# qwerty35/lsc_planner

Hardware: AMD Instinct MI355X
Metric: agent-replans/sec (whole node) (higher is better)
Workload: dtype f64

## Files before the change

### include/lsc_planner_amd.h

```cpp
#ifndef LSC_PLANNER_AMD_H
#define LSC_PLANNER_AMD_H

#include <stddef.h>
#include <stdint.h>

#ifdef __cplusplus
extern "C" {
#endif

#ifndef LSC_SEGMENTS
#define LSC_SEGMENTS 5
#endif
#define LSC_M LSC_SEGMENTS
#define LSC_DEG 5
#define LSC_NC 6
#define LSC_SEGV (LSC_M * LSC_NC)
#define LSC_NV (3 * LSC_SEGV)

#define LSC_OK 0
#define LSC_EINVAL (-1)
#define LSC_ENODEV (-2)
#define LSC_ENOMEM (-3)
#define LSC_EHIP (-4)
#define LSC_ESTATE (-5)
// ... 133 lines not shown

int lsc_gjk_batch(lsc_ctx *ctx, const double *pts, int count, double *v, double *dist);

int lsc_kernel_time_ms(lsc_ctx *ctx, int which, double *avg_ms, long *launches);
int lsc_set_timing(lsc_ctx *ctx, int enabled);
int lsc_kernel_times_ms(lsc_ctx *ctx, int which, double *out_ms, long capacity, long *launches);

int lsc_last_goals(lsc_ctx *ctx, float *goals);
int lsc_goal_storage(lsc_ctx *ctx, int *where);

int lsc_set_goal_trace(lsc_ctx *ctx, int path_cap);
int lsc_get_goal_trace(lsc_ctx *ctx, int *path_cells, int *path_len, int *flags, int *expansions, int grid_dims[3],
                       double grid_min[3]);

int lsc_last_row_counts(lsc_ctx *ctx, int *rows);
int lsc_neighbour_counts(lsc_ctx *ctx, int *units, int *priority_candidates);
int lsc_row_capacity(const lsc_ctx *ctx, int *lds_rows, int *throughput_rows);
int lsc_last_bucket_max(lsc_ctx *ctx, int *rows);

int lsc_iterations_total(lsc_ctx *ctx, long long *total, int reset);
int lsc_row_iterations_total(lsc_ctx *ctx, long long *total);

int lsc_solver_stats(lsc_ctx *ctx, long long out[4]);

int lsc_phase_profile(lsc_ctx *ctx, int enable, long long *out);
int lsc_goal_profile(lsc_ctx *ctx, int enable, long long *out);
int lsc_goal_key_table(int words, unsigned int *out, int *rank_bits);
int lsc_general_profile(lsc_ctx *ctx, long long *out);
int lsc_solver_residuals(lsc_ctx *ctx, double *out);
int lsc_dump_qp(lsc_ctx *ctx, int agent, const char *path);
int lsc_solver_trace(lsc_ctx *ctx, int agent, double *out);

#ifdef __cplusplus
}
#endif
#endif
```

### lsc_planner_amd/_lib.py

```python
import ctypes
import os

_HERE = os.path.dirname(os.path.abspath(__file__))
_LIBS = {}

M, DEG, NC, SEGV, NV = 5, 5, 6, 30, 90


def segments_of(horizon, dt):
    return int((horizon + 1e-9) / dt)

STATUS_OK, STATUS_INFEASIBLE, STATUS_SFC_BLOCKED, STATUS_GOAL_CAPACITY = 0, 1, 4, 5
COMM_ID_BYTES = 128


class LscError(RuntimeError):
    pass


class LscConfig(ctypes.Structure):
    _fields_ = [
        ("dt", ctypes.c_double),
        ("control_weight", ctypes.c_double),
        ("terminal_weight", ctypes.c_double),
# ... 13 lines not shown
        ("grid_resolution", ctypes.c_double),
        ("grid_margin", ctypes.c_double),
        ("horizon", ctypes.c_double),
        ("goal_row_cap", ctypes.c_int),
        ("planner_mode", ctypes.c_int),
        ("slack_mode", ctypes.c_int),
        ("slack_collision_weight", ctypes.c_double),
        ("n_constraint_segments", ctypes.c_int),
        ("reset_threshold", ctypes.c_double),
        ("gap_tolerance", ctypes.c_double),
        ("world_dimension", ctypes.c_int),
        ("world_z_2d", ctypes.c_double),
        ("goal_search", ctypes.c_int),
        ("solver", ctypes.c_int),
        ("goal_lds_row_cap", ctypes.c_int),
    ]


EXPORTS = [
    "lsc_default_config", "lsc_create", "lsc_destroy", "lsc_last_error", "lsc_last_note", "lsc_segments", "lsc_set_agents", "lsc_set_shard",
    "lsc_set_distmap", "lsc_replan_tick", "lsc_tick_device", "lsc_tick_device_fused", "lsc_propagate_device", "lsc_safety_ratio", "lsc_sweep_device", "lsc_sweep_device_f32",
    "lsc_gjk_batch", "lsc_kernel_time_ms", "lsc_kernel_times_ms", "lsc_set_timing", "lsc_last_row_counts", "lsc_iterations_total", "lsc_phase_profile", "lsc_goal_profile", "lsc_goal_key_table", "lsc_general_profile", "lsc_dump_qp", "lsc_solver_residuals", "lsc_solver_trace", "lsc_edt_from_bt", "lsc_free_host", "lsc_last_goals", "lsc_goal_storage", "lsc_set_goal_trace", "lsc_get_goal_trace",
    "lsc_last_bucket_max", "lsc_row_capacity", "lsc_comm_unique_id", "lsc_comm_init", "lsc_comm_info", "lsc_tick_device_sharded", "lsc_replan_tick_all",
    "lsc_row_iterations_total", "lsc_tick_device_fused_batch", "lsc_solver_stats", "lsc_neighbour_counts", "lsc_replan_tick_batch",
    "lsc_flight_weights", "lsc_flight_row_bytes", "lsc_flight_begin", "lsc_flight_reset", "lsc_flight_end", "lsc_fly_device", "lsc_flight_read",
]

FLIGHT_SAMPLES, FLIGHT_SAFETY, FLIGHT_AGENTS = 1, 2, 4
FLIGHT_MAX_TIMES = 64


class LscFlightConfig(ctypes.Structure):
    _fields_ = [("capacity_ticks", ctypes.c_int), ("n_times", ctypes.c_int), ("times", ctypes.c_double * 64), ("what", ctypes.c_int)]


class LscFlightTick(ctypes.Structure):
    _fields_ = [("planner_seq", ctypes.c_int), ("unmet", ctypes.c_int), ("end_unmet", ctypes.c_int), ("moved", ctypes.c_int),
                ("n_status", ctypes.c_int * 6), ("min_ratio", ctypes.c_double), ("pad", ctypes.c_int * 4)]


BUILT_SEGMENTS = (5, 4)


def lib_path(segments=5):
    if segments == 5:
        return os.environ.get("LSC_HIP_LIB") or os.path.join(_HERE, "liblsc_hip.so")
    if segments == 4:
# ... 48 lines not shown
    L.lsc_kernel_times_ms.argtypes = [vp, ctypes.c_int, dp, ctypes.c_long, ctypes.POINTER(ctypes.c_long)]
    L.lsc_set_timing.argtypes = [vp, ctypes.c_int]
    L.lsc_last_row_counts.argtypes = [vp, ip]
    L.lsc_neighbour_counts.argtypes = [vp, ip, ip]
    L.lsc_last_bucket_max.argtypes = [vp, ip]
    L.lsc_row_capacity.argtypes = [vp, ip, ip]
    L.lsc_phase_profile.argtypes = [vp, ctypes.c_int, ctypes.POINTER(ctypes.c_longlong)]
    L.lsc_goal_profile.argtypes = [vp, ctypes.c_int, ctypes.POINTER(ctypes.c_longlong)]
    L.lsc_general_profile.argtypes = [vp, ctypes.POINTER(ctypes.c_longlong)]
    L.lsc_goal_key_table.argtypes = [ctypes.c_int, ctypes.POINTER(ctypes.c_uint), ctypes.POINTER(ctypes.c_int)]
    L.lsc_dump_qp.argtypes = [vp, ctypes.c_int, ctypes.c_char_p]
    L.lsc_solver_residuals.argtypes = [vp, dp]
    L.lsc_solver_trace.argtypes = [vp, ctypes.c_int, dp]
    L.lsc_edt_from_bt.argtypes = [ctypes.c_char_p, fp, fp, ctypes.c_double, ctypes.POINTER(fp), ip, ip, dp]
    L.lsc_last_goals.argtypes = [vp, fp]
    L.lsc_goal_storage.argtypes = [vp, ip]
    L.lsc_set_goal_trace.argtypes = [vp, ctypes.c_int]
    L.lsc_get_goal_trace.argtypes = [vp, ip, ip, ip, ip, ip, dp]
    L.lsc_free_host.argtypes = [vp]
    L.lsc_free_host.restype = None
    L.lsc_iterations_total.argtypes = [vp, ctypes.POINTER(ctypes.c_longlong), ctypes.c_int]
    L.lsc_row_iterations_total.argtypes = [vp, ctypes.POINTER(ctypes.c_longlong)]
    L.lsc_solver_stats.argtypes = [vp, ctypes.POINTER(ctypes.c_longlong)]
    L.lsc_flight_weights.argtypes = [ctypes.c_double, dp, ctypes.c_int, dp, dp, dp, ip]
    L.lsc_flight_row_bytes.argtypes = [ctypes.c_int, ctypes.c_int, ctypes.c_int]
    L.lsc_flight_row_bytes.restype = ctypes.c_size_t
    L.lsc_flight_begin.argtypes = [vp, ctypes.POINTER(LscFlightConfig)]
    L.lsc_flight_reset.argtypes = [vp]
    L.lsc_flight_end.argtypes = [vp]
    L.lsc_fly_device.argtypes = [vp, vpp, vp, vpp, ctypes.c_int, ctypes.c_int, vp, vp, vp, vp]
    L.lsc_flight_read.argtypes = [vp, ctypes.c_int, ctypes.c_int, ctypes.POINTER(LscFlightTick), fp, dp, ip, dp, ip, fp]
    for name in EXPORTS:
        fn = getattr(L, name)
        if fn.restype is ctypes.c_int or name not in ("lsc_default_config", "lsc_create", "lsc_destroy", "lsc_last_error", "lsc_last_note", "lsc_free_host",
                                                      "lsc_flight_row_bytes"):
            fn.restype = ctypes.c_int
    L.lsc_segments.argtypes = []
    if L.lsc_segments() != segments:
        raise LscError(f"{p} plans M = {L.lsc_segments()} segments, not {segments}")
    _LIBS[segments] = L
    return L
```

### lsc_planner_amd/csrc/lsc_abi.cpp

```cpp
#include <hip/hip_runtime.h>
#include <rccl/rccl.h>
#include <dlfcn.h>

#include <cmath>
#include <cstdio>
#include <cstdlib>
#include <cstring>
#include <chrono>
#include <algorithm>
#include <map>
#include <mutex>
#include <string>
#include <unordered_map>
#include <vector>

#include "../../include/lsc_planner_amd.h"
#include "lsc_kernels.h"
#include "lsc_rules.hpp"
#include "lsc_flight.hpp"
#include "lsc_device_mem.hpp"

using namespace lsc;

namespace {
// ... 252 lines not shown
    float *d_state = nullptr, *d_goal = nullptr, *d_prev = nullptr, *d_next = nullptr;
    double *d_cost = nullptr;
    int *d_status = nullptr, *d_iters = nullptr;
    PinnedBuf<float> h_in;
    PinnedBuf<unsigned char> h_out;
    DevBuf<float> d_onormal;
    DevBuf<double> d_od;
    DevBuf<unsigned char> d_spill;
    size_t spill_stride = 0;
    int spill_slots = 0;
    DevBuf<unsigned char> d_ever, d_gen_ws;
    size_t gen_stride = 0;
    int gen_slots = 0;
    DevBuf<unsigned char> d_neigh;
    DevBuf<long long> d_neigh_prof;
    NeighArgs neigh = {};
    DevBuf<unsigned char> d_safety;
    DevBuf<unsigned char> d_flight;
    int flight_capacity = 0, flight_times = 0, flight_what = 0, flight_flown = 0;
    size_t flight_row_bytes = 0;
    hipStream_t flight_stream = nullptr;
    DevBuf<long long> d_goal_prof;
    DevBuf<int> d_goal_path, d_goal_plen;
    MapMem map;
};

static constexpr size_t in_block_floats(size_t n) { return (9 + 3 + NV) * n; }
static constexpr size_t out_block_bytes(size_t rows) { return (sizeof(double) + sizeof(float) * NV + 2 * sizeof(int)) * rows; }
static constexpr size_t FLIGHT_W5 = 0, FLIGHT_W4 = FLIGHT_W5 + 8 * 6 * FLIGHT_MAX_TIMES, FLIGHT_W3 = FLIGHT_W4 + 8 * 5 * FLIGHT_MAX_TIMES,
                        FLIGHT_SEG = FLIGHT_W3 + 8 * 4 * FLIGHT_MAX_TIMES, FLIGHT_HEADER_BYTES = 8192;
static_assert(FLIGHT_SEG + 4 * FLIGHT_MAX_TIMES <= FLIGHT_HEADER_BYTES, "the header holds the tables of 64 record times");
constexpr int TIMED_GROUPS = 7;

struct lsc_ctx {
    lsc_config cfg;
    HostModel hm;
    int N = 0, first = 0, count = 0, cap = 0, cap_tp = 0, n_cu = 256;
    size_t smem_tp = 0;
    std::string err;
    std::string note;
    bool timing = false;
    CtxMem own;
    SwarmMem swarm;
    int last_host_seq = 0;
    bool next_has_all_rows = false;
    bool h_ever_stale = false;
    std::vector<unsigned char> h_ever;
    std::vector<float> h_edt;
    int edt_dims[3] = {0, 0, 0}, edt_kmin[3] = {0, 0, 0};
    double edt_res = 0.0;
    std::vector<double> h_radius;
    int goal_path_cap = 0;
    std::vector<uint32_t> h_fcode;
    int fcode_rb = 0;
    bool goal_profiling = false;
    int grid_dims[3] = {0, 0, 0}, grid_row_cap = 0;
    double grid_min[3] = {0, 0, 0};
    std::vector<int> nb_seq;
    int goal_hbm = 0;
    size_t goal_ws_bytes = 0;
    bool neigh_always = false;
    bool general_handover = false;
    bool generic_lsc_build = false;
    int trace_agent = -1;
    bool profiling = false;
    hipStream_t stream = nullptr;
    std::vector<std::pair<hipEvent_t, hipEvent_t>> ev_pool[TIMED_GROUPS];
    std::vector<double> host_tick_ms;
    size_t ev_used[TIMED_GROUPS] = {0, 0, 0, 0, 0, 0, 0};
    int world = 1, rank = 0, shard_rows = 0, table_rows = 0;
    ncclComm_t comm = nullptr;
};

struct RcclApi {
    void *h = nullptr;
    decltype(&ncclGetUniqueId) GetUniqueId = nullptr;
    decltype(&ncclCommInitRank) CommInitRank = nullptr;
    decltype(&ncclCommDestroy) CommDestroy = nullptr;
    decltype(&ncclAllGather) AllGather = nullptr;
    decltype(&ncclAllReduce) AllReduce = nullptr;
    decltype(&ncclGroupStart) GroupStart = nullptr;
    decltype(&ncclGroupEnd) GroupEnd = nullptr;
    decltype(&ncclGetErrorString) GetErrorString = nullptr;
};

static bool rccl_bind(RcclApi &api);
// ... 230 lines not shown
    if (cap < NBR * (N - 1)) {
        s.spill_stride = plan_spill_bytes(N);
        s.spill_slots = std::min(N, 256);
        HIPCHK(c, s.d_spill.alloc(s.spill_stride * (size_t)s.spill_slots));
    }
    {
        HIPCHK(c, s.d_ever.alloc_zero(n));
        c->h_ever.assign(N, 0);
        const bool general_all = c->cfg.planner_mode == 1 || c->cfg.slack_mode != 0;
        if (general_all || c->cfg.reset_threshold > 0.0) {
            s.gen_stride = general_ws_bytes(N);
            s.gen_slots = std::min(N, 256);
            HIPCHK(c, s.d_gen_ws.alloc(s.gen_stride * (size_t)s.gen_slots));
        }
        c->general_handover = getenv("LSC_GENERAL_HANDOVER") != nullptr;
    }
    {
        c->generic_lsc_build = getenv("LSC_GENERIC_LSC_BUILD") != nullptr;
        const size_t prev = c->note.find("lsc build:");
        if (prev != std::string::npos) c->note.erase(prev >= 2 ? prev - 2 : prev);
        const char *which = c->generic_lsc_build ? "generic pass (LSC_GENERIC_LSC_BUILD)"
                            : (N - 1 > 64 ? "generic pass (more than 64 obstacles)" : "one wave per segment");
        c->note += (c->note.empty() ? "" : "; ") + std::string("lsc build: ") + which;
    }
    HIPCHK(c, s.d_nrows.alloc_zero(n));
    HIPCHK(c, s.d_bmax.alloc_zero(n));
    HIPCHK(c, s.d_order.alloc(n));
    HIPCHK(c, s.d_obs_bound.alloc(4 * n));
    if (N >= NEIGH_MIN_AGENTS && N <= NEIGH_MAX_AGENTS && c->cfg.prune == 1 && !getenv("LSC_NO_NEIGHBOUR_LISTS")) {
        NeighArgs &g = s.neigh;
        c->neigh_always = getenv("LSC_NEIGH_ALWAYS") != nullptr;
        double vm = 0.0, rm = 0.0, dmin = 1e300, dmax = 0.0;
        for (int i = 0; i < N; i++) {
            for (int k = 0; k < 3; k++) vm = std::max(vm, max_vel[3 * i + k]);
            rm = std::max(rm, radius[i]); dmin = std::min(dmin, dw_obs[i]); dmin = std::min(dmin, downwash[i]);
            dmax = std::max(dmax, dw_obs[i]); dmax = std::max(dmax, downwash[i]);
        }
        double cell = vm * M * c->cfg.dt + 4.0 * rm;
        if (const char *e = getenv("LSC_NEIGH_CELL")) { const double v = atof(e); if (v > 0.0) cell = v; }
        if (!(cell > 1e-3)) cell = 1e-3;
        g.sc_max = std::max(1.0, 1.0 / dmin); g.zscale = std::max(1.0, dmax);
        g.inv_cell = 1.0 / cell; g.inv_cell_z = 1.0 / (cell * g.zscale);
        unsigned H = 1024;
        while (H < 4u * (unsigned)N) H <<= 1;
        g.hmask = H - 1; g.ovf_cap = 4096; g.list_cap = 1024; g.plist_cap = NEIGH_PRIO_CAP; g.tag = 0;
        if (const char *e = getenv("LSC_NEIGH_OVF_CAP")) { const int v = atoi(e); if (v >= 1 && v <= 65536) g.ovf_cap = v; }
// ... 395 lines not shown
    a.neigh = c->swarm.neigh.cnt ? &c->swarm.neigh : nullptr;
    a.nv = nullptr;
    a.state = d_state; a.goal = d_goal; a.traj_prev = d_prev;
    a.radius = c->swarm.d_radius; a.radius_obs = c->swarm.d_radius_obs; a.downwash = c->swarm.d_downwash; a.downwash_obs = c->swarm.d_downwash_obs;
    a.vmax = c->swarm.d_vmax; a.amax = c->swarm.d_amax; a.vnom = c->swarm.d_vnom;
    a.traj_next = d_next; a.cost = d_cost; a.status = d_status; a.iters = d_iters; a.nrows = c->swarm.d_nrows; a.bucket_max = c->swarm.d_bmax; a.iters_acc = c->swarm.d_iters_acc;
    a.stale = c->swarm.d_stale; a.sfc = c->cfg.use_octomap ? c->swarm.d_sfc.get() : nullptr;
    a.sfc_err = c->cfg.use_octomap ? c->swarm.d_sfc_err.get() : nullptr;
    const bool planned = c->cfg.goal_mode == 1 && c->cfg.use_octomap;
    a.goal_err = planned ? c->swarm.map.d_goal_err.get() : nullptr;
    a.out_normal = nullptr; a.out_d = nullptr;
    a.goal_mode = planned ? 0 : c->cfg.goal_mode; a.goal_threshold = c->cfg.goal_threshold;
    a.priority_dist_threshold = c->cfg.priority_dist_threshold; a.goal_radius = c->cfg.goal_radius;
    a.goal_out = c->swarm.d_goal_cur; a.state_next = nullptr; a.finv = (float)std::pow(c->cfg.dt, -1);
    a.dbg = c->swarm.d_dbg; a.prof = c->profiling ? c->swarm.d_prof.get() : nullptr;
    a.trace = c->trace_agent >= 0 ? c->own.d_trace.get() : nullptr; a.trace_agent = c->trace_agent;
    a.spill_ws = c->swarm.d_spill; a.spill_stride = c->swarm.spill_stride;
    a.gmodel = c->own.d_gmodel; a.planner_mode = c->cfg.planner_mode; a.slack_mode = c->cfg.slack_mode;
    a.ncs = c->cfg.n_constraint_segments; a.general_all = (c->cfg.planner_mode == 1 || c->cfg.slack_mode != 0) ? 1 : 0;
    a.slack_w = c->cfg.slack_collision_weight; a.reset_thr = c->cfg.planner_mode == 0 ? c->cfg.reset_threshold : 0.0;
    a.ever = c->swarm.d_ever; a.gen_ws = c->swarm.d_gen_ws; a.gen_stride = c->swarm.gen_stride;
    a.fold = 0;
    a.generic_lsc_build = c->generic_lsc_build ? 1 : 0;
    return LSC_OK;
}

static bool want_general(const lsc_ctx *c, int general_hint)
{
    if (!c->swarm.d_gen_ws) return false;
    if (c->cfg.planner_mode == 1 || c->cfg.slack_mode != 0) return true;
    return general_hint != 0;
}

static int host_disturbance_hint(lsc_ctx *c, const float *state, const float *prev_traj, int planner_seq)
{
    if (!(c->cfg.reset_threshold > 0.0) || c->cfg.planner_mode != 0) return 0;
    if (c->h_ever_stale) {
        if (c->swarm.d_ever && !c->h_ever.empty() &&
            (hipDeviceSynchronize() != hipSuccess ||
             hipMemcpy(c->h_ever.data(), c->swarm.d_ever, c->h_ever.size(), hipMemcpyDeviceToHost) != hipSuccess)) return 1;
        c->h_ever_stale = false;
    }
    int any = 0;
    for (int q = 0; q < c->N; q++) {
        if (planner_seq >= 2) {
            const float *t = prev_traj + (size_t)q * NV + NC;
// ... 1009 lines not shown
int lsc_row_iterations_total(lsc_ctx *c, long long *total)
{
    if (!c || !total || c->N == 0) return LSC_EINVAL;
    std::vector<long long> h(c->N);
    HIPCHK(c, hipDeviceSynchronize());
    HIPCHK(c, hipMemcpy(h.data(), c->swarm.d_iters_acc + c->N, sizeof(long long) * (size_t)c->N, hipMemcpyDeviceToHost));
    long long t = 0;
    for (long long v : h) t += v;
    *total = t;
    return LSC_OK;
}

int lsc_solver_stats(lsc_ctx *c, long long out[4])
{
    if (!c || !out || c->N == 0) return LSC_EINVAL;
    HIPCHK(c, hipDeviceSynchronize());
    std::vector<long long> h(4 * (size_t)c->N);
    HIPCHK(c, hipMemcpy(h.data(), c->swarm.d_iters_acc + 2 * (size_t)c->N, sizeof(long long) * h.size(), hipMemcpyDeviceToHost));
    for (int k = 0; k < 4; k++) out[k] = 0;
    for (int q = 0; q < c->N; q++) for (int k = 0; k < 4; k++) out[k] += h[4 * (size_t)q + k];
    return LSC_OK;
}

int lsc_set_goal_trace(lsc_ctx *c, int path_cap)
{
    if (!c || c->N == 0 || path_cap < 0) return LSC_EINVAL;
    c->swarm.d_goal_path.reset();
    c->swarm.d_goal_plen.reset();
    c->goal_path_cap = path_cap;
    if (path_cap > 0) {
        HIPCHK(c, c->swarm.d_goal_path.alloc((size_t)c->N * path_cap));
        HIPCHK(c, c->swarm.d_goal_plen.alloc_zero((size_t)c->N));
    }
    return LSC_OK;
}

int lsc_get_goal_trace(lsc_ctx *c, int *path_cells, int *path_len, int *flags, int *expansions, int grid_dims[3],
                       double grid_min[3])
{
    if (!c || c->N == 0) return LSC_EINVAL;
    if (!c->swarm.map.d_goal_flags) { c->err = "goal trace: the goal planner is not active (goal_mode 1 + use_octomap + distmap)"; return LSC_ESTATE; }
    HIPCHK(c, hipDeviceSynchronize());
    const size_t cnt = c->count, first = c->first;
    if (flags) HIPCHK(c, hipMemcpy(flags, c->swarm.map.d_goal_flags + first, sizeof(int) * cnt, hipMemcpyDeviceToHost));
    if (expansions) HIPCHK(c, hipMemcpy(expansions, c->swarm.map.d_goal_exp + first, sizeof(int) * cnt, hipMemcpyDeviceToHost));
    if (grid_dims) for (int k = 0; k < 3; k++) grid_dims[k] = c->grid_dims[k];
// ... 75 lines not shown
```

### lsc_planner_amd/csrc/lsc_kernels.h

```cpp
#pragma once
#include <hip/hip_runtime.h>
#include <hip/hip_ext.h>
#include <stddef.h>
#include <stdint.h>

#include "lsc_model.hpp"

#define LSC_STATUS_OK_K 0
#define LSC_STATUS_INFEASIBLE_K 1
#define LSC_STATUS_CAPACITY_K 3
#define LSC_STATUS_SFC_K 4
#define LSC_STATUS_GOAL_K 5
#define LSC_STATUS_GENERAL_K 6

namespace lsc {

struct PlanArgs;
struct NeighArgs;
struct NeighView;
#if defined(__HIP_DEVICE_COMPILE__)
typedef const __attribute__((address_space(4))) PlanArgs KArgs;
#else
typedef const PlanArgs KArgs;
#endif
// ... 33 lines not shown
    const float *sfc;
    const int *sfc_err;
    const int *goal_err;
    float *out_normal;
    double *out_d;
    double *dbg;
    long long *prof;
    double *trace;
    int trace_agent;
    unsigned char *spill_ws;
    size_t spill_stride;
    const GModel *gmodel;
    int planner_mode;
    int slack_mode;
    int ncs;
    int general_all;
    double slack_w;
    double reset_thr;
    unsigned char *ever;
    unsigned char *gen_ws;
    size_t gen_stride;
    int fold;
    int generic_lsc_build;
};
constexpr int PROF_PHASES = 16;
constexpr int LDS_MAX_BYTES = 160 * 1024;

inline bool plan_alt_hooks(const PlanArgs &a) { return a.general_all || (a.reset_thr > 0.0 && a.ever); }

struct KernelVariant {
    int key;
    const void *fn;
};
template <class... A>
inline const void *kernel_address(void (*f)(A...)) { return reinterpret_cast<const void *>(f); }
template <size_t n>
inline const void *find_variant(const KernelVariant (&table)[n], int key)
{
    for (const KernelVariant &v : table)
        if (v.key == key) return v.fn;
    return nullptr;
}
template <size_t n>
inline hipError_t allow_full_lds(const KernelVariant (&table)[n])
{
    for (const KernelVariant &v : table) {
// ... 225 lines not shown
```

### lsc_planner_amd/csrc/lsc_kernels.hip

```cpp
#include <hip/hip_runtime.h>
#include <math.h>
#include <stdint.h>

#include "lsc_general.hpp"
#include "lsc_gjk.hpp"
#include "lsc_model.hpp"
#include "lsc_kernels.h"
#include "lsc_rules.hpp"
#include "lsc_wave.hpp"

namespace lsc {

constexpr int NT = 512;
constexpr int NWAVE = NT / 64;

template <bool F32>
__global__ __launch_bounds__(256) void lsc_sweep_kernel(SweepArgs a)
{
    const int n_obs = a.N - 1;
    const long total = (long)a.count * n_obs * M;
    for (long u = (long)blockIdx.x * blockDim.x + threadIdx.x; u < total; u += (long)gridDim.x * blockDim.x) {
        const int m = (int)(u % M);
        const int oi = (int)((u / M) % n_obs);
        const int al = (int)(u / ((long)M * n_obs));
        const int qi = a.first + al;
// ... 439 lines not shown
}

constexpr int TW_A = (NY - BAND + 1) / 2;
constexpr int TW_B = NY - BAND - TW_A;
constexpr int TW_M1 = NY - TW_B;
static_assert(TW_M1 - TW_A == BAND, "the middle block must absorb exactly one bandwidth");

template <int J, int JEND>
__device__ __forceinline__ void fwd_steps(const double (&rowS)[TW_M1], double &b)
{
    const double bj = bcast_lane<J>(b);
    b = fma(-rowS[J], bj, b);
    if constexpr (J + 1 < JEND) fwd_steps<J + 1, JEND>(rowS, b);
}
template <int I, int LO, int CNT>
__device__ __forceinline__ void bwd_steps(const double (&c)[CNT], double &b)
{
    const double xi = bcast_lane<I>(b);
    b = fma(-c[I - LO], xi, b);
    if constexpr (I > LO) bwd_steps<I - 1, LO, CNT>(c, b);
}

#define LSC_P(a, i) "+v"(a[i])
__device__ __forceinline__ void pin_values(double (&a)[8])
{
    asm volatile("" : LSC_P(a, 0), LSC_P(a, 1), LSC_P(a, 2), LSC_P(a, 3), LSC_P(a, 4), LSC_P(a, 5), LSC_P(a, 6), LSC_P(a, 7));
}
__device__ __forceinline__ void pin_values(double (&a)[9])
{
    asm volatile("" : LSC_P(a, 0), LSC_P(a, 1), LSC_P(a, 2), LSC_P(a, 3), LSC_P(a, 4), LSC_P(a, 5), LSC_P(a, 6), LSC_P(a, 7), LSC_P(a, 8));
}
__device__ __forceinline__ void pin_values(double (&a)[10])
{
    asm volatile("" : LSC_P(a, 0), LSC_P(a, 1), LSC_P(a, 2), LSC_P(a, 3), LSC_P(a, 4), LSC_P(a, 5), LSC_P(a, 6), LSC_P(a, 7), LSC_P(a, 8), LSC_P(a, 9));
}
__device__ __forceinline__ void pin_values(double (&a)[11])
{
    asm volatile("" : LSC_P(a, 0), LSC_P(a, 1), LSC_P(a, 2), LSC_P(a, 3), LSC_P(a, 4), LSC_P(a, 5), LSC_P(a, 6), LSC_P(a, 7), LSC_P(a, 8), LSC_P(a, 9),
                 LSC_P(a, 10));
}
__device__ __forceinline__ void pin_values(double (&a)[12])
{
    asm volatile("" : LSC_P(a, 0), LSC_P(a, 1), LSC_P(a, 2), LSC_P(a, 3), LSC_P(a, 4), LSC_P(a, 5), LSC_P(a, 6), LSC_P(a, 7), LSC_P(a, 8), LSC_P(a, 9), LSC_P(a, 10), LSC_P(a, 11));
}
__device__ __forceinline__ void pin_values(double (&a)[13])
{
// ... 1372 lines not shown
        static_assert(GQ * GS + GQ * GQ + 2 * GQ + (GQ + 1) / 2 <= NY * KLD, "the working set fits the idle K");
        double *const gyv = S.gz;
        double *const gi_hz = S.as_;
        double *const gi_zt = S.az;
        static_assert(SEGV * NYA <= AXROWS, "gi_hz fits the slack array");
        const double INF = 1e300;
        if (!early) {
#pragma unroll
        for (int u = 0; u < GI_NPRE; u++) if (tid + u * NT < SEGV * NYA) { gi_hz[tid + u * NT] = gi_pre_z[u]; gi_zt[tid + u * NT] = gi_pre_n[u]; }
        }
        if (!early) for (int c = tid; c < n_ax; c += NT) { const int sl = S.amap[c] & 1023; S.at2[sl] = rcp_nr(1.0 + fabs(AH(sl))); }
        for (int c = tid; c < nact; c += NT) { const int r = cmap[c] & CMAP_MASK; rt2[r] = rcp_nr(1.0 + fabs(rrhs[r])); }
        if (!early) {
        for (int i = tid; i < GQ * GS + GQ * GQ + 2 * GQ; i += NT) Yw[i] = 0.0;
        if (tid < 40) {
            const int k = tid < NY ? yaxis(tid) : 0;
            double yv = gi_pre_y[0] * S.s0[k][0] + gi_pre_y[1] * S.s0[k][1] + gi_pre_y[2] * S.s0[k][2] + gi_pre_y[3] * S.goal[k];
            if (dim2 && k == 2) yv = md.z2d;
            S.y[tid] = tid < NY ? yv : 0.0;
        }
        __syncthreads();
        }
        int q = 0;
        const int xv0 = lane, xv1 = lane + 64 < NV ? lane + 64 : lane;
        const uint32_t xg0 = S.xgp[xv0], xg1 = S.xgp[xv1];
        const double xa00 = S.xtc[xv0 % SEGV][0], xa01 = S.xtc[xv0 % SEGV][1], xa02 = S.xtc[xv0 % SEGV][2];
        const double xa10 = S.xtc[xv1 % SEGV][0], xa11 = S.xtc[xv1 % SEGV][1], xa12 = S.xtc[xv1 % SEGV][2];
        const bool xs0 = xv0 % SEGV < 3, xs1 = xv1 % SEGV < 3;
        const double xk0 = xs0 ? X0C(xv0) : 0.0, xk1 = xs1 ? X0C(xv1) : 0.0;
        auto gi_x = [&]() { gi_x_lanes(xv0, xv1, xg0, xg1, xa00, xa01, xa02, xa10, xa11, xa12, xs0, xs1, xk0, xk1); };
        if (!early) {
            if (wave == 0) gi_x();
            __syncthreads();
        }
        stamp(PH_INIT);
        const bool s_has_ax = tid < n_ax, s_has_l = tid < nact;
        const uint32_t s_am = S.amap[s_has_ax ? tid : 0];
        const int s_sl = s_am & 1023, s_type = (s_am >> 10) & 7, s_xo = (int)((s_am >> 13) & 3) * SEGV + (int)(s_am >> 15);
        const double s_hh = AH(s_sl);
        const uint32_t s_e = s_has_l ? cmap[tid] : 0u;
        const int s_r = s_e & CMAP_MASK, s_cp = s_e >> CMAP_SHIFT;
        const double s_lh = rrhs[s_r];
        const float s_n0 = rn[s_r], s_n1 = rn[R + s_r], s_n2 = rn[2 * R + s_r];
        for (;;) {
            double best = 0.0;
            int bidx = 0;
// ... 12 lines not shown
                double sc = S.at2[sl], x0 = xq[0], x1 = xq[1], x2 = xq[2], hh = AH(sl);
                LSC_PIN(PV(sc), PV(x0), PV(x1), PV(x2), PV(hh));
                const double v = (ax_row3(x0, x1, x2, type) - hh) * sc;
                if (v > best) { best = v; bidx = c; }
            }
            if (s_has_l && lv > best) { best = lv; bidx = n_ax + tid; }
            for (int c = tid + NT; c < nact; c += NT) {
                const uint32_t e = cmap[c];
                const int r = e & CMAP_MASK, cp = e >> CMAP_SHIFT;
                double sc = rt2[r], x0 = S.x[cp], x1 = S.x[SEGV + cp], x2 = S.x[2 * SEGV + cp], hh = rrhs[r];
                float n0 = rn[r], n1 = rn[R + r], n2 = rn[2 * R + r];
                LSC_PIN(PV(sc), PV(x0), PV(x1), PV(x2), PV(hh), PV(n0), PV(n1), PV(n2));
                const double v = (hh - ((double)n0 * x0 + (double)n1 * x1 + (double)n2 * x2)) * sc;
                if (v > best) { best = v; bidx = n_ax + c; }
            }
            const unsigned long long key = best > 0.0 ? (((unsigned long long)__float_as_uint((float)best)) << 32) | (unsigned long long)(0xffffffffu - (uint32_t)bidx) : 0ull;
            block_reduce(__longlong_as_double((long long)key), 0.0, 0.0, 0.0, 0.0, 1, -1, -1, -1, -1);
            const unsigned long long kmax = (unsigned long long)__double_as_longlong(rv[0]);
            stamp(PH_P1);
            if (!(__uint_as_float((uint32_t)(kmax >> 32)) > 1e-10f)) break;
            const int idx = (int)(0xffffffffu - (uint32_t)(kmax & 0xffffffffull));
            if (wave == 0) {
                q = __builtin_amdgcn_readfirstlane(q);
                int v0, v1, v2, rsl = 0;
                double a0, a1, a2, hp;
                auto uni = [](bool b_) { return __builtin_amdgcn_readfirstlane((int)b_) != 0; };
                const bool is_ax = idx < n_ax;
                if (is_ax) {
                    const uint32_t am = S.amap[idx]; const int sl = am & 1023, type = (am >> 10) & 7, ak = (am >> 13) & 3, at = am >> 15;
                    const int kind = type >> 1;
                    const double sg = (type & 1) ? -1.0 : 1.0;
                    a0 = sg * (kind == 1 ? -1.0 : 1.0); a1 = sg * (kind == 0 ? 0.0 : (kind == 1 ? 1.0 : -2.0)); a2 = sg * (kind == 2 ? 1.0 : 0.0);
                    v0 = ak * SEGV + at; v1 = kind >= 1 ? v0 + 1 : v0; v2 = kind == 2 ? v0 + 2 : v0;
                    rsl = sl;
                } else {
                    const uint32_t e = cmap[idx - n_ax];
                    const int r = e & CMAP_MASK, cp = e >> CMAP_SHIFT;
                    v0 = cp; v1 = SEGV + cp; v2 = 2 * SEGV + cp;
                    rsl = r;
                    a0 = a1 = a2 = 0.0;
                }
                const int t0 = v0 % SEGV, t1 = v1 % SEGV, t2 = v2 % SEGV, k0 = v0 / SEGV, k1 = v1 / SEGV, k2 = v2 / SEGV;
                const int lk = lane < NY ? yaxis(lane) : 3, lva = lane < NY ? yvar(lane) : 0;
                {
                    double hh = is_ax ? AH(rsl) : -rrhs[rsl];
                    float n0 = 0.f, n1 = 0.f, n2 = 0.f;
                    if (!is_ax) { n0 = rn[rsl]; n1 = rn[R + rsl]; n2 = rn[2 * R + rsl]; }
                    LSC_PIN(PV(hh), PV(n0), PV(n1), PV(n2));
                    hp = hh;
                    if (!is_ax) { a0 = -(double)n0; a1 = -(double)n1; a2 = -(double)n2; }
                }
                double x0 = S.x[v0], x1 = S.x[v1], x2 = S.x[v2];
                uint32_t gp0 = S.xgp[v0], gp1 = S.xgp[v1], gp2 = S.xgp[v2];
                double c00 = S.xtc[t0][0], c01 = S.xtc[t0][1], c02 = S.xtc[t0][2], c10 = S.xtc[t1][0], c11 = S.xtc[t1][1], c12 = S.xtc[t1][2],
                       c20 = S.xtc[t2][0], c21 = S.xtc[t2][1], c22 = S.xtc[t2][2];
                double h0 = gi_hz[t0 * NYA + lva], h1 = gi_hz[t1 * NYA + lva], h2 = gi_hz[t2 * NYA + lva];
                double z0 = gi_zt[t0 * NYA + lva], z1 = gi_zt[t1 * NYA + lva], z2 = gi_zt[t2 * NYA + lva];
                LSC_PIN(PV(x0), PV(x1), PV(x2), PV(gp0), PV(gp1), PV(gp2), PV(c00), PV(c01), PV(c02), PV(c10), PV(c11), PV(c12), PV(c20), PV(c21), PV(c22),
                        PV(h0), PV(h1), PV(h2), PV(z0), PV(z1), PV(z2));
                double viol = a0 * x0 + a1 * x1 + a2 * x2 - hp;
                const double m0 = lk == k0 ? a0 : 0.0, m1 = lk == k1 ? a1 : 0.0, m2 = lk == k2 ? a2 : 0.0;
                const double np_g = m0 * z0 + m1 * z1 + m2 * z2;
                double hin_g = m0 * h0 + m1 * h1 + m2 * h2;
                if (dim2 && lk == 2) hin_g = 0.0;
                double up = 0.0;
                int code = 0;
                const int lq = lane < GQ ? lane : GQ - 1, lg = lane < GS ? lane : GS - 1;
                for (;;) {
                    __builtin_amdgcn_fence(__ATOMIC_RELEASE, "wavefront");
                    __builtin_amdgcn_wave_barrier();
                    __builtin_amdgcn_fence(__ATOMIC_ACQUIRE, "wavefront");
                    double Sr[GQ], Yc[GQ];
                    const double *yr = Yw + lq * GS;
                    double y00 = yr[gp0 & 0xff], y01 = yr[(gp0 >> 8) & 0xff], y02 = yr[gp0 >> 16], y10 = yr[gp1 & 0xff], y11 = yr[(gp1 >> 8) & 0xff], y12 = yr[gp1 >> 16],
                           y20 = yr[gp2 & 0xff], y21 = yr[(gp2 >> 8) & 0xff], y22 = yr[gp2 >> 16];
#pragma unroll
                    for (int j = 0; j < GQ; j++) { Sr[j] = Si[lq * GQ + j]; Yc[j] = Yw[j * GS + lg]; }
                    double uwl = uw[lq], yl = S.y[lg];
                    LSC_PIN(PV(y00), PV(y01), PV(y02), PV(y10), PV(y11), PV(y12), PV(y20), PV(y21), PV(y22), PV(uwl), PV(yl));
                    pin_values(Sr);
                    pin_values(Yc);
                    double dw = a0 * (c00 * y00 + c01 * y01 + c02 * y02) + a1 * (c10 * y10 + c11 * y11 + c12 * y12) + a2 * (c20 * y20 + c21 * y21 + c22 * y22);
                    dw = lane < q ? dw : 0.0;
                    double rw = 0.0;
#pragma unroll
                    for (int j = 0; j < GQ; j++) rw = fma(Sr[j], lane_value(dw, j), rw);
                    rw = lane < q ? rw : 0.0;
                    if (lane < GQ) rwv[lane] = rw;
                    double rb[GQ];
#pragma unroll
                    for (int w = 0; w < GQ; w++) rb[w] = rwv[w];
                    pin_values(rb);
                    double zg = hin_g;
#pragma unroll
                    for (int w = 0; w < GQ; w++) zg = fma(-Yc[w], rb[w], zg);
                    zg = lane < NY ? zg : 0.0;
                    const double ratio = (lane < q && rw > 1e-13) ? uwl * rcp_nr(rw) : INF;
                    double red4[5] = {np_g * hin_g, np_g * zg, ratio, 0.0, 0.0};
                    const int rop[5] = {0, 0, 2, -1, -1};
                    wave_reduce5(red4, rop);
                    const double nph = red4[0], zn = red4[1], t1 = red4[2];
                    const unsigned long long dropmask = __ballot(lane < q && ratio == t1);
                    const double t2 = zn > 1e-12 * nph ? viol * rcp_nr(zn) : INF;
                    if (uni(t1 >= INF && t2 >= INF)) {
                        code = uni(viol > 1e-6 * (1.0 + fabs(hp))) ? 3 : 1;
                        break;
                    }
                    const double t = fmin(t1, t2);
                    if (uni(t2 < INF)) {
                        if (lane < NY) S.y[lane] = yl - t * zg;
                        viol -= t * zn;
                    }
                    if (lane < q) uw[lane] = fmax(uwl - t * rw, 0.0);
                    up += t;
                    gi_changes++;
                    if (uni(t2 <= t1)) {
                        if (uni(q == GQ)) { code = 2; break; }
                        const double delta = zn;
                        if (uni(!(delta > 1e-11 * nph))) { code = 2; break; }
                        const double idl = rcp_nr(delta);
                        if (lane < GS) Yw[q * GS + lane] = hin_g;
                        const double rs_ = rw * idl;
#pragma unroll
                        for (int j = 0; j < GQ; j++) Sr[j] = fma(rs_, rb[j], Sr[j]);
                        if (lane < q) {
#pragma unroll
                            for (int j = 0; j < GQ; j++) Si[lane * GQ + j] = Sr[j];
                            Si[lane * GQ + q] = -rs_;
                            Si[q * GQ + lane] = -rs_;
                        }
                        if (lane == 0) {
                            Si[q * GQ + q] = idl; uw[q] = up; wrow[q] = idx;
                            if (is_ax) S.at2[rsl] = 0.0;
                            else rt2[rsl] = 0.0;
                        }
                        q = __builtin_amdgcn_readfirstlane(q + 1);
                        break;
                    }
                    const int jd = __builtin_amdgcn_readfirstlane(__ffsll((long long)dropmask) - 1), last = q - 1;
                    if (lane == 0) {
                        const int code_j = wrow[jd];
                        if (code_j < n_ax) { const int sl = S.amap[code_j] & 1023; S.at2[sl] = rcp_nr(1.0 + fabs(AH(sl))); }
                        else { const int r = cmap[code_j - n_ax] & CMAP_MASK; rt2[r] = rcp_nr(1.0 + fabs(rrhs[r])); }
                    }
                    {
                        const double cjj = Si[jd * GQ + jd];
                        const double bi = Si[lq * GQ + jd] * (1.0 / cjj);
                        double Tn[GQ];
#pragma unroll
                        for (int k = 0; k < GQ; k++) Tn[k] = fma(-bi, Si[jd * GQ + k], Sr[k]);
                        pin_values(Tn);
                        if (lane < q && lane != jd) {
                            const int ir = lane == last ? jd : lane;
#pragma unroll
                            for (int k = 0; k < GQ; k++) {
                                if (k < q && k != jd) Si[ir * GQ + (k == last ? jd : k)] = Tn[k];
                            }
                        }
                    }
                    if (uni(jd != last)) {
                        if (lane < GS) Yw[jd * GS + lane] = Yw[last * GS + lane];
                        if (lane == 0) { uw[jd] = uw[last]; wrow[jd] = wrow[last]; }
                    }
                    q = __builtin_amdgcn_readfirstlane(q - 1);
                    gi_changes = __builtin_amdgcn_readfirstlane(gi_changes);
                    if (uni(gi_changes > GI_CAP)) { code = 2; break; }
                }
                if (uni(code == 3)) {
                    gi_x();
                    __builtin_amdgcn_fence(__ATOMIC_RELEASE, "wavefront");
                    __builtin_amdgcn_wave_barrier();
                    __builtin_amdgcn_fence(__ATOMIC_ACQUIRE, "wavefront");
                    auto residual = [&](int rc) -> double {
                        if (rc < n_ax) {
                            const uint32_t am = S.amap[rc]; const int sl = am & 1023, type = (am >> 10) & 7, ak = (am >> 13) & 3, at = am >> 15;
                            const double *xq = S.x + ak * SEGV + at;
                            return ax_row3(xq[0], xq[1], xq[2], type) - AH(sl);
                        }
                        const uint32_t e = cmap[rc - n_ax];
                        const int r = e & CMAP_MASK, cp = e >> CMAP_SHIFT;
                        return rrhs[r] - ((double)rn[r] * S.x[cp] + (double)rn[R + r] * S.x[SEGV + cp] + (double)rn[2 * R + r] * S.x[2 * SEGV + cp]);
                    };
                    const double rj = lane < q ? rwv[lane] : 0.0;
                    const double part = lane < q ? rj * residual(wrow[lane]) : 0.0;
                    const double gap = residual(idx) - wave_sum(part);
                    if (uni(!(gap > 0.5e-6 * (1.0 + fabs(hp))))) code = 1;
                }
                if (lane == 0) { S.sc[0] = (double)code; S.sc[1] = (double)q; S.sc[2] = (double)gi_changes; }
                if (code == 0) gi_x();
            }
            __syncthreads();
            stamp(PH_FACTOR);
            if (S.sc[0] != 0.0) { gi_infeasible = S.sc[0] == 3.0; return false; }
            q = (int)S.sc[1];
            gi_changes = (int)S.sc[2];
        }
        {
            double worst = 0.0;
            for (int c = tid; c < n_ax; c += NT) {
                const uint32_t am = S.amap[c]; const int sl = am & 1023, type = (am >> 10) & 7, ak = (am >> 13) & 3, at = am >> 15;
                const double *xq = S.x + ak * SEGV + at;
                double x0 = xq[0], x1 = xq[1], x2 = xq[2], hh = AH(sl);
                LSC_PIN(PV(x0), PV(x1), PV(x2), PV(hh));
                worst = fmax(worst, (ax_row3(x0, x1, x2, type) - hh) * rcp_nr(1.0 + fabs(hh)));
            }
            for (int c = tid; c < nact; c += NT) {
                const uint32_t e = cmap[c];
                const int r = e & CMAP_MASK, cp = e >> CMAP_SHIFT;
                double x0 = S.x[cp], x1 = S.x[SEGV + cp], x2 = S.x[2 * SEGV + cp], hh = rrhs[r];
                float n0 = rn[r], n1 = rn[R + r], n2 = rn[2 * R + r];
                LSC_PIN(PV(x0), PV(x1), PV(x2), PV(hh), PV(n0), PV(n1), PV(n2));
                worst = fmax(worst, (hh - ((double)n0 * x0 + (double)n1 * x1 + (double)n2 * x2)) * rcp_nr(1.0 + fabs(hh)));
            }
            double objp = 0.0;
            if (tid < NV && !(dim2 && xk == 2)) {
                objp = 0.5 * cost_grad() * S.x[tid];
                if (xterm) { const double e = S.x[tid] - S.goal[xk]; objp += md.w_t * e * e; }
            }
            block_reduce(worst, objp, 0.0, 0.0, 0.0, 1, 0, -1, -1, -1);
            if (rv[0] > 1e-9) return false;
            obj = rv[1];
        }
        stamp(PH_P2);
        return true;
        }
    };

    bool run = true, run_gi_done = false;
    if (a.goal_err && a.goal_err[qi] != 0) {
        status = LSC_STATUS_GOAL_K;
        run = false;
    } else if (a.sfc_err && a.sfc_err[qi] != 0) {
        status = LSC_STATUS_SFC_K;
        run = false;
    } else if (ALT && S.gen) {
        status = LSC_STATUS_GENERAL_K;
        run = false;
    } else if (overflow) {
        status = LSC_STATUS_CAPACITY_K;
        run = false;
    } else if (SOLVER == 1 && gi_solve() && a.solver != 2) {
        status = LSC_STATUS_OK_K;
// ... 703 lines not shown
```

### lsc_planner_amd/planner.py

```python
import ctypes
import os
from dataclasses import dataclass, field

import numpy as np

from . import _lib
from ._lib import LscConfig, LscError, M, NC, NV, SEGV


@dataclass
class PlannerConfig:
    dt: float = 0.2
    control_input_weight: float = 0.01
    terminal_weight: float = 1.0
    use_octomap: bool = False
    world_resolution: float = 0.1
    device: int = 0
    max_rows_per_cp: int = 0
    max_iters: int = 50
    prune: bool = True
    warm_start_mu: float = 0.03
    goal_mode: str = "static"
    goal_threshold: float = 0.1
    priority_dist_threshold: float = 0.4
# ... 358 lines not shown
        wsz = 3 * self.NV + 6 * self.SEGV
        out = np.zeros(64 * 8 + ny * kld + wsz + 512)
        self._check(self.L.lsc_solver_trace(self.ctx, agent, _dp(out) if read else None))
        self.trace_K = out[512:512 + ny * kld].reshape(ny, kld)[:, :ny]
        self.trace_W = out[512 + ny * kld:512 + ny * kld + wsz]
        self.trace_kconst = out[512 + ny * kld + wsz:]
        return out[:512].reshape(64, 8)

    def iterations_total(self, reset=False):
        t = ctypes.c_longlong()
        self._check(self.L.lsc_iterations_total(self.ctx, ctypes.byref(t), int(reset)))
        return t.value

    def row_iterations_total(self):
        t = ctypes.c_longlong()
        self._check(self.L.lsc_row_iterations_total(self.ctx, ctypes.byref(t)))
        return t.value

    def solver_stats(self):
        out = (ctypes.c_longlong * 4)()
        self._check(self.L.lsc_solver_stats(self.ctx, out))
        return dict(solved=out[0], handed_over=out[1], changes=out[2], ip_iterations=out[3])

    def set_timing(self, on):
        self._check(self.L.lsc_set_timing(self.ctx, int(on)))

    def kernel_time_ms(self, which=0):
        ms = ctypes.c_double()
        n = ctypes.c_long()
        self._check(self.L.lsc_kernel_time_ms(self.ctx, which, ctypes.byref(ms), ctypes.byref(n)))
        return ms.value, n.value

    def kernel_times_ms(self, which=0):
        n = ctypes.c_long()
        self._check(self.L.lsc_kernel_times_ms(self.ctx, which, None, 0, ctypes.byref(n)))
        out = np.zeros(max(n.value, 1), np.float64)
        self._check(self.L.lsc_kernel_times_ms(self.ctx, which, out.ctypes.data_as(ctypes.POINTER(ctypes.c_double)), n.value,
                                               ctypes.byref(n)))
        return out[:n.value]


def tick_device_fused_batch(planners, states, goals, trajs_prev, trajs_next, states_next, costs, statuses, iters, planner_seqs, stream=0):
    n = len(planners)
    L = planners[0].L
    if not all(p.L is L for p in planners):
        raise LscError("tick_device_fused_batch: planners of different libraries (segment counts) in one batch")
# ... 84 lines not shown
```

Measured before the change: 1.622 million.

## Specialise Goldfarb-Idnani change step by working-set size class

The active-set change loop in the dual QP solver is templated on a compile-time slot count (4, 8 or GQ) and dispatched by the running working-set high-water mark. Unrolled loops and register arrays then cover only the slots in use rather than the full GQ capacity, which cuts FMAs, LDS reads and register pressure for small working sets. Segment/axis indices are also computed directly instead of via modulo/division. It adds code size from three instantiations, an env-var fallback, and an optional per-agent peak-tracking debug buffer.

Result: faster. 1.675 million (median of 6 runs) (+3.2%).

```diff
diff --git a/include/lsc_planner_amd.h b/include/lsc_planner_amd.h
--- a/include/lsc_planner_amd.h
+++ b/include/lsc_planner_amd.h
@@ -179,6 +179,7 @@
 int lsc_row_iterations_total(lsc_ctx *ctx, long long *total);
 
 int lsc_solver_stats(lsc_ctx *ctx, long long out[4]);
+int lsc_working_set_peaks(lsc_ctx *ctx, int *peaks);
 
 int lsc_phase_profile(lsc_ctx *ctx, int enable, long long *out);
 int lsc_goal_profile(lsc_ctx *ctx, int enable, long long *out);
diff --git a/lsc_planner_amd/_lib.py b/lsc_planner_amd/_lib.py
--- a/lsc_planner_amd/_lib.py
+++ b/lsc_planner_amd/_lib.py
@@ -59,7 +59,7 @@
     "lsc_set_distmap", "lsc_replan_tick", "lsc_tick_device", "lsc_tick_device_fused", "lsc_propagate_device", "lsc_safety_ratio", "lsc_sweep_device", "lsc_sweep_device_f32",
     "lsc_gjk_batch", "lsc_kernel_time_ms", "lsc_kernel_times_ms", "lsc_set_timing", "lsc_last_row_counts", "lsc_iterations_total", "lsc_phase_profile", "lsc_goal_profile", "lsc_goal_key_table", "lsc_general_profile", "lsc_dump_qp", "lsc_solver_residuals", "lsc_solver_trace", "lsc_edt_from_bt", "lsc_free_host", "lsc_last_goals", "lsc_goal_storage", "lsc_set_goal_trace", "lsc_get_goal_trace",
     "lsc_last_bucket_max", "lsc_row_capacity", "lsc_comm_unique_id", "lsc_comm_init", "lsc_comm_info", "lsc_tick_device_sharded", "lsc_replan_tick_all",
-    "lsc_row_iterations_total", "lsc_tick_device_fused_batch", "lsc_solver_stats", "lsc_neighbour_counts", "lsc_replan_tick_batch",
+    "lsc_row_iterations_total", "lsc_tick_device_fused_batch", "lsc_solver_stats", "lsc_working_set_peaks", "lsc_neighbour_counts", "lsc_replan_tick_batch",
     "lsc_flight_weights", "lsc_flight_row_bytes", "lsc_flight_begin", "lsc_flight_reset", "lsc_flight_end", "lsc_fly_device", "lsc_flight_read",
 ]
 
@@ -154,6 +154,7 @@
     L.lsc_iterations_total.argtypes = [vp, ctypes.POINTER(ctypes.c_longlong), ctypes.c_int]
     L.lsc_row_iterations_total.argtypes = [vp, ctypes.POINTER(ctypes.c_longlong)]
     L.lsc_solver_stats.argtypes = [vp, ctypes.POINTER(ctypes.c_longlong)]
+    L.lsc_working_set_peaks.argtypes = [vp, ip]
     L.lsc_flight_weights.argtypes = [ctypes.c_double, dp, ctypes.c_int, dp, dp, dp, ip]
     L.lsc_flight_row_bytes.argtypes = [ctypes.c_int, ctypes.c_int, ctypes.c_int]
     L.lsc_flight_row_bytes.restype = ctypes.c_size_t
diff --git a/lsc_planner_amd/csrc/lsc_abi.cpp b/lsc_planner_amd/csrc/lsc_abi.cpp
--- a/lsc_planner_amd/csrc/lsc_abi.cpp
+++ b/lsc_planner_amd/csrc/lsc_abi.cpp
@@ -298,6 +298,7 @@
     hipStream_t flight_stream = nullptr;
     DevBuf<long long> d_goal_prof;
     DevBuf<int> d_goal_path, d_goal_plen;
+    DevBuf<int> d_ws_peak;
     MapMem map;
 };
 
@@ -338,6 +339,7 @@
     bool neigh_always = false;
     bool general_handover = false;
     bool generic_lsc_build = false;
+    bool step_all_slots = false;
     int trace_agent = -1;
     bool profiling = false;
     hipStream_t stream = nullptr;
@@ -614,6 +616,8 @@
         const char *which = c->generic_lsc_build ? "generic pass (LSC_GENERIC_LSC_BUILD)"
                             : (N - 1 > 64 ? "generic pass (more than 64 obstacles)" : "one wave per segment");
         c->note += (c->note.empty() ? "" : "; ") + std::string("lsc build: ") + which;
+        c->step_all_slots = getenv("LSC_STEP_ALL_SLOTS") != nullptr;
+        c->note += std::string("; step: ") + (c->step_all_slots ? "all slots (LSC_STEP_ALL_SLOTS)" : "size classes");
     }
     HIPCHK(c, s.d_nrows.alloc_zero(n));
     HIPCHK(c, s.d_bmax.alloc_zero(n));
@@ -1055,6 +1059,8 @@
     a.ever = c->swarm.d_ever; a.gen_ws = c->swarm.d_gen_ws; a.gen_stride = c->swarm.gen_stride;
     a.fold = 0;
     a.generic_lsc_build = c->generic_lsc_build ? 1 : 0;
+    a.step_all_slots = c->step_all_slots ? 1 : 0;
+    a.ws_peak = c->swarm.d_ws_peak;
     return LSC_OK;
 }
 
@@ -2110,6 +2116,15 @@
     return LSC_OK;
 }
 
+int lsc_working_set_peaks(lsc_ctx *c, int *peaks )
+{
+    if (!c || !peaks || c->N == 0) return LSC_EINVAL;
+    HIPCHK(c, hipDeviceSynchronize());
+    if (!c->swarm.d_ws_peak) HIPCHK(c, c->swarm.d_ws_peak.alloc_zero((size_t)c->N));
+    HIPCHK(c, hipMemcpy(peaks, c->swarm.d_ws_peak, sizeof(int) * (size_t)c->N, hipMemcpyDeviceToHost));
+    return LSC_OK;
+}
+
 int lsc_set_goal_trace(lsc_ctx *c, int path_cap)
 {
     if (!c || c->N == 0 || path_cap < 0) return LSC_EINVAL;
diff --git a/lsc_planner_amd/csrc/lsc_kernels.h b/lsc_planner_amd/csrc/lsc_kernels.h
--- a/lsc_planner_amd/csrc/lsc_kernels.h
+++ b/lsc_planner_amd/csrc/lsc_kernels.h
@@ -79,6 +79,8 @@
     size_t gen_stride;
     int fold;
     int generic_lsc_build;
+    int step_all_slots;
+    int *ws_peak;
 };
 constexpr int PROF_PHASES = 16;
 constexpr int LDS_MAX_BYTES = 160 * 1024;
diff --git a/lsc_planner_amd/csrc/lsc_kernels.hip b/lsc_planner_amd/csrc/lsc_kernels.hip
--- a/lsc_planner_amd/csrc/lsc_kernels.hip
+++ b/lsc_planner_amd/csrc/lsc_kernels.hip
@@ -1,6 +1,8 @@
 #include <hip/hip_runtime.h>
 #include <math.h>
 #include <stdint.h>
+
+#include <type_traits>
 
 #include "lsc_general.hpp"
 #include "lsc_gjk.hpp"
@@ -486,6 +488,10 @@
 }
 
 #define LSC_P(a, i) "+v"(a[i])
+__device__ __forceinline__ void pin_values(double (&a)[4])
+{
+    asm volatile("" : LSC_P(a, 0), LSC_P(a, 1), LSC_P(a, 2), LSC_P(a, 3));
+}
 __device__ __forceinline__ void pin_values(double (&a)[8])
 {
     asm volatile("" : LSC_P(a, 0), LSC_P(a, 1), LSC_P(a, 2), LSC_P(a, 3), LSC_P(a, 4), LSC_P(a, 5), LSC_P(a, 6), LSC_P(a, 7));
@@ -1904,6 +1910,9 @@
         __syncthreads();
         }
         int q = 0;
+        int qhw = 0;
+        const bool all_slots = a.step_all_slots != 0;
+        auto peak_out = [&]() { if (a.ws_peak && tid == 0) a.ws_peak[qi] = qhw; };
         const int xv0 = lane, xv1 = lane + 64 < NV ? lane + 64 : lane;
         const uint32_t xg0 = S.xgp[xv0], xg1 = S.xgp[xv1];
         const double xa00 = S.xtc[xv0 % SEGV][0], xa01 = S.xtc[xv0 % SEGV][1], xa02 = S.xtc[xv0 % SEGV][2];
@@ -1962,7 +1971,7 @@
             const int idx = (int)(0xffffffffu - (uint32_t)(kmax & 0xffffffffull));
             if (wave == 0) {
                 q = __builtin_amdgcn_readfirstlane(q);
-                int v0, v1, v2, rsl = 0;
+                int v0, v1, v2, t0, t1, t2, k0, k1, k2, rsl = 0;
                 double a0, a1, a2, hp;
                 auto uni = [](bool b_) { return __builtin_amdgcn_readfirstlane((int)b_) != 0; };
                 const bool is_ax = idx < n_ax;
@@ -1972,15 +1981,18 @@
                     const double sg = (type & 1) ? -1.0 : 1.0;
                     a0 = sg * (kind == 1 ? -1.0 : 1.0); a1 = sg * (kind == 0 ? 0.0 : (kind == 1 ? 1.0 : -2.0)); a2 = sg * (kind == 2 ? 1.0 : 0.0);
                     v0 = ak * SEGV + at; v1 = kind >= 1 ? v0 + 1 : v0; v2 = kind == 2 ? v0 + 2 : v0;
+                    t0 = at; t1 = kind >= 1 ? at + 1 : at; t2 = kind == 2 ? at + 2 : at;
+                    k0 = k1 = k2 = ak;
                     rsl = sl;
                 } else {
                     const uint32_t e = cmap[idx - n_ax];
                     const int r = e & CMAP_MASK, cp = e >> CMAP_SHIFT;
                     v0 = cp; v1 = SEGV + cp; v2 = 2 * SEGV + cp;
+                    t0 = t1 = t2 = cp;
+                    k0 = 0; k1 = 1; k2 = 2;
                     rsl = r;
                     a0 = a1 = a2 = 0.0;
                 }
-                const int t0 = v0 % SEGV, t1 = v1 % SEGV, t2 = v2 % SEGV, k0 = v0 / SEGV, k1 = v1 / SEGV, k2 = v2 / SEGV;
                 const int lk = lane < NY ? yaxis(lane) : 3, lva = lane < NY ? yvar(lane) : 0;
                 {
                     double hh = is_ax ? AH(rsl) : -rrhs[rsl];
@@ -2006,16 +2018,18 @@
                 double up = 0.0;
                 int code = 0;
                 const int lq = lane < GQ ? lane : GQ - 1, lg = lane < GS ? lane : GS - 1;
-                for (;;) {
+                auto change = [&](auto qc_) -> bool {
+                    constexpr int QC = decltype(qc_)::value;
+                    static_assert(QC <= GQ, "a class is a prefix of the working set's slots");
                     __builtin_amdgcn_fence(__ATOMIC_RELEASE, "wavefront");
                     __builtin_amdgcn_wave_barrier();
                     __builtin_amdgcn_fence(__ATOMIC_ACQUIRE, "wavefront");
-                    double Sr[GQ], Yc[GQ];
+                    double Sr[QC], Yc[QC];
                     const double *yr = Yw + lq * GS;
                     double y00 = yr[gp0 & 0xff], y01 = yr[(gp0 >> 8) & 0xff], y02 = yr[gp0 >> 16], y10 = yr[gp1 & 0xff], y11 = yr[(gp1 >> 8) & 0xff], y12 = yr[gp1 >> 16],
                            y20 = yr[gp2 & 0xff], y21 = yr[(gp2 >> 8) & 0xff], y22 = yr[gp2 >> 16];
 #pragma unroll
-                    for (int j = 0; j < GQ; j++) { Sr[j] = Si[lq * GQ + j]; Yc[j] = Yw[j * GS + lg]; }
+                    for (int j = 0; j < QC; j++) { Sr[j] = Si[lq * GQ + j]; Yc[j] = Yw[j * GS + lg]; }
                     double uwl = uw[lq], yl = S.y[lg];
                     LSC_PIN(PV(y00), PV(y01), PV(y02), PV(y10), PV(y11), PV(y12), PV(y20), PV(y21), PV(y22), PV(uwl), PV(yl));
                     pin_values(Sr);
@@ -2024,16 +2038,16 @@
                     dw = lane < q ? dw : 0.0;
                     double rw = 0.0;
 #pragma unroll
-                    for (int j = 0; j < GQ; j++) rw = fma(Sr[j], lane_value(dw, j), rw);
+                    for (int j = 0; j < QC; j++) rw = fma(Sr[j], lane_value(dw, j), rw);
                     rw = lane < q ? rw : 0.0;
                     if (lane < GQ) rwv[lane] = rw;
-                    double rb[GQ];
-#pragma unroll
-                    for (int w = 0; w < GQ; w++) rb[w] = rwv[w];
+                    double rb[QC];
+#pragma unroll
+                    for (int w = 0; w < QC; w++) rb[w] = rwv[w];
                     pin_values(rb);
                     double zg = hin_g;
 #pragma unroll
-                    for (int w = 0; w < GQ; w++) zg = fma(-Yc[w], rb[w], zg);
+                    for (int w = 0; w < QC; w++) zg = fma(-Yc[w], rb[w], zg);
                     zg = lane < NY ? zg : 0.0;
                     const double ratio = (lane < q && rw > 1e-13) ? uwl * rcp_nr(rw) : INF;
                     double red4[5] = {np_g * hin_g, np_g * zg, ratio, 0.0, 0.0};
@@ -2044,7 +2058,7 @@
                     const double t2 = zn > 1e-12 * nph ? viol * rcp_nr(zn) : INF;
                     if (uni(t1 >= INF && t2 >= INF)) {
                         code = uni(viol > 1e-6 * (1.0 + fabs(hp))) ? 3 : 1;
-                        break;
+                        return true;
                     }
                     const double t = fmin(t1, t2);
                     if (uni(t2 < INF)) {
@@ -2055,17 +2069,17 @@
                     up += t;
                     gi_changes++;
                     if (uni(t2 <= t1)) {
-                        if (uni(q == GQ)) { code = 2; break; }
+                        if (uni(q == GQ)) { code = 2; qhw = GQ + 1; return true; }
                         const double delta = zn;
-                        if (uni(!(delta > 1e-11 * nph))) { code = 2; break; }
+                        if (uni(!(delta > 1e-11 * nph))) { code = 2; return true; }
                         const double idl = rcp_nr(delta);
                         if (lane < GS) Yw[q * GS + lane] = hin_g;
                         const double rs_ = rw * idl;
 #pragma unroll
-                        for (int j = 0; j < GQ; j++) Sr[j] = fma(rs_, rb[j], Sr[j]);
+                        for (int j = 0; j < QC; j++) Sr[j] = fma(rs_, rb[j], Sr[j]);
                         if (lane < q) {
 #pragma unroll
-                            for (int j = 0; j < GQ; j++) Si[lane * GQ + j] = Sr[j];
+                            for (int j = 0; j < QC; j++) Si[lane * GQ + j] = Sr[j];
                             Si[lane * GQ + q] = -rs_;
                             Si[q * GQ + lane] = -rs_;
                         }
@@ -2075,7 +2089,8 @@
                             else rt2[rsl] = 0.0;
                         }
                         q = __builtin_amdgcn_readfirstlane(q + 1);
-                        break;
+                        qhw = __builtin_amdgcn_readfirstlane(q > qhw ? q : qhw);
+                        return true;
                     }
                     const int jd = __builtin_amdgcn_readfirstlane(__ffsll((long long)dropmask) - 1), last = q - 1;
                     if (lane == 0) {
@@ -2086,14 +2101,14 @@
                     {
                         const double cjj = Si[jd * GQ + jd];
                         const double bi = Si[lq * GQ + jd] * (1.0 / cjj);
-                        double Tn[GQ];
-#pragma unroll
-                        for (int k = 0; k < GQ; k++) Tn[k] = fma(-bi, Si[jd * GQ + k], Sr[k]);
+                        double Tn[QC];
+#pragma unroll
+                        for (int k = 0; k < QC; k++) Tn[k] = fma(-bi, Si[jd * GQ + k], Sr[k]);
                         pin_values(Tn);
                         if (lane < q && lane != jd) {
                             const int ir = lane == last ? jd : lane;
 #pragma unroll
-                            for (int k = 0; k < GQ; k++) {
+                            for (int k = 0; k < QC; k++) {
                                 if (k < q && k != jd) Si[ir * GQ + (k == last ? jd : k)] = Tn[k];
                             }
                         }
@@ -2104,7 +2119,16 @@
                     }
                     q = __builtin_amdgcn_readfirstlane(q - 1);
                     gi_changes = __builtin_amdgcn_readfirstlane(gi_changes);
-                    if (uni(gi_changes > GI_CAP)) { code = 2; break; }
+                    if (uni(gi_changes > GI_CAP)) { code = 2; return true; }
+                    return false;
+                };
+                for (;;) {
+                    const int qn = all_slots ? GQ : qhw;
+                    bool over;
+                    if (qn <= 4) over = change(std::integral_constant<int, 4>());
+                    else if (qn <= 8 || GQ <= 8) over = change(std::integral_constant<int, GQ < 8 ? GQ : 8>());
+                    else over = change(std::integral_constant<int, GQ>());
+                    if (over) break;
                 }
                 if (uni(code == 3)) {
                     gi_x();
@@ -2131,7 +2155,7 @@
             }
             __syncthreads();
             stamp(PH_FACTOR);
-            if (S.sc[0] != 0.0) { gi_infeasible = S.sc[0] == 3.0; return false; }
+            if (S.sc[0] != 0.0) { gi_infeasible = S.sc[0] == 3.0; peak_out(); return false; }
             q = (int)S.sc[1];
             gi_changes = (int)S.sc[2];
         }
@@ -2158,6 +2182,7 @@
                 if (xterm) { const double e = S.x[tid] - S.goal[xk]; objp += md.w_t * e * e; }
             }
             block_reduce(worst, objp, 0.0, 0.0, 0.0, 1, 0, -1, -1, -1);
+            peak_out();
             if (rv[0] > 1e-9) return false;
             obj = rv[1];
         }
diff --git a/lsc_planner_amd/planner.py b/lsc_planner_amd/planner.py
--- a/lsc_planner_amd/planner.py
+++ b/lsc_planner_amd/planner.py
@@ -404,6 +404,11 @@
         self._check(self.L.lsc_solver_stats(self.ctx, out))
         return dict(solved=out[0], handed_over=out[1], changes=out[2], ip_iterations=out[3])
 
+    def working_set_peaks(self):
+        out = np.zeros(self.N, np.int32)
+        self._check(self.L.lsc_working_set_peaks(self.ctx, _ip(out)))
+        return out
+
     def set_timing(self, on):
         self._check(self.L.lsc_set_timing(self.ctx, int(on)))
 
```
